# evenrose/CMDIAD

Measured on AMD Instinct MI355X. Metric: images/sec end-to-end (extract+distill+kNN score), higher is better.
Workload: dtype bf16; 1 GPU; configs[1]: DINO ViT-B/8 + Point-MAE predict (DoubleRGBPointFeatures: both modalities are extracted, this method has no distillation step at test time; the `mtfi_step` leg times the method that has one), 224x224 RGB + 24576-point clouds (1024 groups x 128), batch 32/GPU, bagel-sized banks (xyz 76518x768, rgb 19129x768); batch_per_gpu=32, rotating_input_batches=4, bank=single, hip_graphs=True, search_operands=bf16 (fp32 accumulate, exact fp32 re-score of the winner), weights=seeded random init (no checkpoints offline)

## Files before the change

### cmdiad_amd/csrc/mlp_fused.hip

```cpp
#include "gemm_core.h"
#include "launch.h"

namespace {

using namespace gemm;

constexpr int kC = 384, kHid = 1536, kBM = 128, kWaves = 8;
constexpr int kChunks = kHid / 64;
constexpr int kKT1 = kC / BK;
constexpr int kPer = kKT1 + kC / 64;
constexpr int kSlots = 6, kAhead = kSlots - 1;
static_assert(kPer % kSlots == 0, "the slot of a piece depends on its place in the chunk only");
constexpr int kPieceBytes = 64 * BK * 2;
constexpr int kXbWave = kKT1 * 16 * BK * 2;
constexpr int kHOff = kWaves * kXbWave;
constexpr int kRingOff = kHOff + kWaves * 2048;
constexpr int kLdsBytes = kRingOff + kSlots * kPieceBytes;
static_assert(kLdsBytes == 160 * 1024, "LDS budget");

struct MlpParams {
    int M;
    const bf16_t* xb;
    const float* row_scale;
    const bf16_t* w1;
    const float* b1;
    const bf16_t* w2;
    const float* b2;
    float* x;
    bf16_t* ln_xb;
    float* ln_part;
    const float* add2;
};

__device__ __forceinline__ void mlp_barrier() { asm volatile("s_barrier" ::: "memory"); }

__device__ __forceinline__ float half_row_sum8(float v)
{
    v += __builtin_bit_cast(float, __builtin_amdgcn_update_dpp(0, __builtin_bit_cast(int, v), 0xB1, 0xF, 0xF, false));
    v += __builtin_bit_cast(float, __builtin_amdgcn_update_dpp(0, __builtin_bit_cast(int, v), 0x4E, 0xF, 0xF, false));
    v += __builtin_bit_cast(float, __builtin_amdgcn_update_dpp(0, __builtin_bit_cast(int, v), 0x141, 0xF, 0xF, false));
    return v;
}

template <bool LN_OUT>
__global__ __launch_bounds__(512, 1) void pmae_mlp_fused_kernel(MlpParams p)
{
    extern __shared__ __attribute__((aligned(16))) char lds[];
    const int lane = threadIdx.x & 63, wave = __builtin_amdgcn_readfirstlane(threadIdx.x >> 6);
    const int g = lane >> 4, r16 = lane & 15;
    const int mw = (int)blockIdx.x * kBM + wave * 16;
    char* xs = lds + wave * kXbWave;
    char* hs = lds + kHOff + wave * 2048;
    char* ring = lds + kRingOff;

    float rsc;
    f32x4 b1v[4];
    auto load_b1 = [&](int c) {
        const float* bp = p.b1 + c * 64 + g * 4;
#pragma unroll
        for (int j = 0; j < 4; ++j) asm volatile("global_load_dwordx4 %0, %1, off" : "=v"(b1v[j]) : "v"(bp + j * 16) : "memory");
    };
    {
        const float* rp = p.row_scale + min(mw + r16, p.M - 1);
        asm volatile("global_load_dword %0, %1, off" : "=v"(rsc) : "v"(rp) : "memory");
    }
    load_b1(0);
    const int sw_chunk = (lane & 7) ^ (lane >> 3);
#pragma unroll
    for (int e = 0; e < 2; ++e) {
        const bf16_t* src = p.xb + (size_t)min(mw + e * 8 + (lane >> 3), p.M - 1) * kC + sw_chunk * 8;
#pragma unroll
        for (int s = 0; s < kKT1; ++s)
            __builtin_amdgcn_global_load_lds((const __attribute__((address_space(1))) void*)(src + s * BK),
                                             (__attribute__((address_space(3))) void*)(xs + s * 2048 + e * 1024), 16, 0, 0);
    }
    const char* w1l = reinterpret_cast<const char*>(p.w1 + (size_t)(wave * 8 + (lane >> 3)) * kC + sw_chunk * 8);
    const char* w2l = reinterpret_cast<const char*>(p.w2 + (size_t)(wave * 8 + (lane >> 3)) * kHid + sw_chunk * 8);
    auto issue = [&](int c, int q) {
        const char* src = q < kKT1 ? w1l + ((size_t)c * 64 * kC + q * BK) * 2 : w2l + ((size_t)(q - kKT1) * 64 * kHid + c * BK) * 2;
        __builtin_amdgcn_global_load_lds((const __attribute__((address_space(1))) void*)src,
                                         (__attribute__((address_space(3))) void*)(ring + (q % kSlots) * kPieceBytes + wave * 1024), 16, 0, 0);
    };
#pragma unroll
    for (int q = 0; q < kAhead; ++q) issue(0, q);
    asm volatile("s_waitcnt vmcnt(4)" ::: "memory");
    mlp_barrier();

    auto ldf = [&](const char* tile, int row, int kk) { return *reinterpret_cast<const bf16x8*>(tile + lds_off(row, kk * 4 + g)); };
    auto step = [&](const char* wt, const bf16x8& a0, const bf16x8& a1, f32x4 (&acc)[4]) {
        bf16x8 wf[2][4];
#pragma unroll
        for (int kk = 0; kk < 2; ++kk)
#pragma unroll
            for (int j = 0; j < 4; ++j) wf[kk][j] = ldf(wt, j * 16 + r16, kk);
        __builtin_amdgcn_s_setprio(1);
#pragma unroll
        for (int kk = 0; kk < 2; ++kk)
#pragma unroll
            for (int j = 0; j < 4; ++j) acc[j] = mfma16(wf[kk][j], kk ? a1 : a0, acc[j]);
        __builtin_amdgcn_s_setprio(0);
    };

    f32x4 acc2[kC / 64][4];
#pragma unroll
    for (int nb = 0; nb < kC / 64; ++nb)
#pragma unroll
        for (int j = 0; j < 4; ++j) acc2[nb][j] = f32x4{0.f, 0.f, 0.f, 0.f};

    for (int c = 0; c < kChunks; ++c) {
        f32x4 acc1[4];
#pragma unroll
        for (int j = 0; j < 4; ++j) acc1[j] = f32x4{0.f, 0.f, 0.f, 0.f};
        bf16x8 h0, h1;
#pragma unroll
        for (int q = 0; q < kPer; ++q) {
            const int qn = q + kAhead < kPer ? q + kAhead : q + kAhead - kPer;
            const int cn = q + kAhead < kPer ? c : c + 1;
            const bool more = cn < kChunks;
            if (q == 7 && more) load_b1(c + 1);
            if (more) issue(cn, qn);
            const char* wt = ring + (q % kSlots) * kPieceBytes;
            if (q < kKT1) step(wt, ldf(xs + q * 2048, r16, 0), ldf(xs + q * 2048, r16, 1), acc1);
            else step(wt, h0, h1, acc2[q - kKT1]);
            if (!more) asm volatile("s_waitcnt vmcnt(0)" ::: "memory");
            else if (q >= 7 && q <= 10) asm volatile("s_waitcnt vmcnt(8)" ::: "memory");
            else asm volatile("s_waitcnt vmcnt(4)" ::: "memory");
            mlp_barrier();
            if (q == kKT1 - 1) {
                __builtin_amdgcn_sched_barrier(0);
#pragma unroll
                for (int j = 0; j < 4; ++j) {
                    f32x4 v = __builtin_elementwise_fma(acc1[j], f32x4{rsc, rsc, rsc, rsc}, b1v[j]);
                    v = gelu_erf4(v);
                    const bf16x4 hv = {f2bf(v[0]), f2bf(v[1]), f2bf(v[2]), f2bf(v[3])};
                    *reinterpret_cast<bf16x4*>(hs + lds_off(r16, 2 * j + (g >> 1)) + (g & 1) * 8) = hv;
                }
                h0 = ldf(hs, r16, 0);
                h1 = ldf(hs, r16, 1);
            }
        }
    }

    RowStore32 rs;
    rs.init(hs, lane);
    const bool full = mw + 16 <= p.M;
    const int m0r = mw + rs.R;
    const int ma = min(m0r, p.M - 1), mb = min(m0r + 8, p.M - 1);
#pragma unroll
    for (int nb = 0; nb < kC / 64; ++nb) {
        const int n0 = nb * 64;
        f32x4 bj[4];
#pragma unroll
        for (int j = 0; j < 4; ++j) bj[j] = *reinterpret_cast<const f32x4*>(p.b2 + n0 + j * 16 + g * 4);
        f32x4 o0[2], o1[2];
#pragma unroll
        for (int ch = 0; ch < 2; ++ch) {
            const int col = n0 + ch * 32 + rs.u * 4;
            const f32x4 r0 = *reinterpret_cast<const f32x4*>(p.x + (size_t)ma * kC + col);
            const f32x4 r1 = *reinterpret_cast<const f32x4*>(p.x + (size_t)mb * kC + col);
            f32x4 a0 = {0.f, 0.f, 0.f, 0.f}, a1 = a0;
            if (LN_OUT && p.add2) {
                a0 = *reinterpret_cast<const f32x4*>(p.add2 + (size_t)ma * kC + col);
                a1 = *reinterpret_cast<const f32x4*>(p.add2 + (size_t)mb * kC + col);
            }
            rs.park(acc2[nb][2 * ch] + bj[2 * ch], acc2[nb][2 * ch + 1] + bj[2 * ch + 1]);
            f32x4 t0, t1;
            rs.fetch(t0, t1);
            o0[ch] = t0 + r0;
            o1[ch] = t1 + r1;
            if (LN_OUT && p.add2) { o0[ch] += a0; o1[ch] += a1; }
            if (full || m0r < p.M) *reinterpret_cast<f32x4*>(p.x + (size_t)m0r * kC + col) = o0[ch];
            if (full || m0r + 8 < p.M) *reinterpret_cast<f32x4*>(p.x + (size_t)(m0r + 8) * kC + col) = o1[ch];
            if constexpr (LN_OUT) {
                const bf16x4 v0 = {f2bf(o0[ch][0]), f2bf(o0[ch][1]), f2bf(o0[ch][2]), f2bf(o0[ch][3])};
                const bf16x4 v1 = {f2bf(o1[ch][0]), f2bf(o1[ch][1]), f2bf(o1[ch][2]), f2bf(o1[ch][3])};
                if (full || m0r < p.M) *reinterpret_cast<bf16x4*>(p.ln_xb + (size_t)m0r * kC + col) = v0;
                if (full || m0r + 8 < p.M) *reinterpret_cast<bf16x4*>(p.ln_xb + (size_t)(m0r + 8) * kC + col) = v1;
            }
        }
        if constexpr (LN_OUT) {
            float s0 = 0.f, s1 = 0.f;
#pragma unroll
            for (int ch = 0; ch < 2; ++ch)
#pragma unroll
                for (int q = 0; q < 4; ++q) { s0 += o0[ch][q]; s1 += o1[ch][q]; }
            s0 = half_row_sum8(s0);
            s1 = half_row_sum8(s1);
            const float c0 = s0 * (1.0f / 64), c1 = s1 * (1.0f / 64);
            float q0 = 0.f, q1 = 0.f;
#pragma unroll
            for (int ch = 0; ch < 2; ++ch)
#pragma unroll
                for (int q = 0; q < 4; ++q) {
                    const float d0 = o0[ch][q] - c0, d1 = o1[ch][q] - c1;
                    q0 = fmaf(d0, d0, q0);
                    q1 = fmaf(d1, d1, q1);
                }
            q0 = half_row_sum8(q0);
            q1 = half_row_sum8(q1);
            if (rs.u == 0) {
                float2* part = reinterpret_cast<float2*>(p.ln_part) + (size_t)nb * p.M;
                if (full || m0r < p.M) part[m0r] = make_float2(s0, q0);
                if (full || m0r + 8 < p.M) part[m0r + 8] = make_float2(s1, q1);
            }
        }
    }
}

}

int cmdiad_pmae_mlp_fused(float* x, const uint16_t* xb, const float* rstd, const uint16_t* w1, const float* b1, const uint16_t* w2,
                          const float* b2, int M, uint16_t* ln_xb, float* ln_part, const float* add2, cmdiad_stream_t stream)
{
    CMDIAD_REQUIRE(x && xb && rstd && w1 && b1 && w2 && b2 && M > 0, CMDIAD_ERR_ARG, "cmdiad_pmae_mlp_fused: null operand");
    CMDIAD_REQUIRE(aligned16(x) && aligned16(xb) && aligned16(w1) && aligned16(w2) && aligned16(b1) && aligned16(b2) && (!add2 || aligned16(add2)), CMDIAD_ERR_ARG,
                   "cmdiad_pmae_mlp_fused: operands must be 16-byte aligned");
    CMDIAD_REQUIRE(!ln_xb == !ln_part && (ln_xb || !add2) && (!ln_xb || (((uintptr_t)ln_xb & 7) == 0 && ((uintptr_t)ln_part & 7) == 0)),
                   CMDIAD_ERR_ARG, "cmdiad_pmae_mlp_fused: ln_xb and ln_part come together (8-byte aligned); add2 only with them");
    MlpParams p{M, (const bf16_t*)xb, rstd, (const bf16_t*)w1, b1, (const bf16_t*)w2, b2, x, (bf16_t*)ln_xb, ln_part, add2};
    const dim3 grid((unsigned)((M + kBM - 1) / kBM)), block(kWaves * 64);
    const int rc = ln_xb ? launch_lds<pmae_mlp_fused_kernel<true>>("cmdiad_pmae_mlp_fused", grid, block, kLdsBytes, (hipStream_t)stream, p)
                         : launch_lds<pmae_mlp_fused_kernel<false>>("cmdiad_pmae_mlp_fused", grid, block, kLdsBytes, (hipStream_t)stream, p);
    if (rc) return rc;
    CMDIAD_CHECK_LAUNCH();
    return CMDIAD_OK;
}
```

Before: 1593 images/s.

## Restructure fused Point-MAE MLP to 4 waves of 32 rows with register double-buffering

```diff
diff --git a/cmdiad_amd/csrc/mlp_fused.hip b/cmdiad_amd/csrc/mlp_fused.hip
--- a/cmdiad_amd/csrc/mlp_fused.hip
+++ b/cmdiad_amd/csrc/mlp_fused.hip
@@ -5,16 +5,19 @@
 
 using namespace gemm;
 
-constexpr int kC = 384, kHid = 1536, kBM = 128, kWaves = 8;
+constexpr int kC = 384, kHid = 1536, kBM = 128, kWaves = 4;
+constexpr int kRows = kBM / kWaves;
 constexpr int kChunks = kHid / 64;
 constexpr int kKT1 = kC / BK;
 constexpr int kPer = kKT1 + kC / 64;
-constexpr int kSlots = 6, kAhead = kSlots - 1;
-static_assert(kPer % kSlots == 0, "the slot of a piece depends on its place in the chunk only");
+constexpr int kSlots = 6;
+static_assert(kPer % kSlots == 0 && kPer % 2 == 0, "the slot and the fragment set of a piece depend on its place in the chunk only");
 constexpr int kPieceBytes = 64 * BK * 2;
-constexpr int kXbWave = kKT1 * 16 * BK * 2;
+constexpr int kXbTile = kRows * BK * 2;
+constexpr int kXbWave = kKT1 * kXbTile;
+constexpr int kHWave = kRows * BK * 2;
 constexpr int kHOff = kWaves * kXbWave;
-constexpr int kRingOff = kHOff + kWaves * 2048;
+constexpr int kRingOff = kHOff + kWaves * kHWave;
 constexpr int kLdsBytes = kRingOff + kSlots * kPieceBytes;
 static_assert(kLdsBytes == 160 * 1024, "LDS budget");
 
@@ -32,7 +35,20 @@
     const float* add2;
 };
 
-__device__ __forceinline__ void mlp_barrier() { asm volatile("s_barrier" ::: "memory"); }
+__device__ __forceinline__ void step_end(int n)
+{
+#define CMDIAD_STEP_END(N) asm volatile("s_waitcnt vmcnt(" #N ") lgkmcnt(0)\n\ts_barrier" ::: "memory")
+    __builtin_amdgcn_s_waitcnt(0xC07F);
+    switch (n) {
+    case 12: CMDIAD_STEP_END(12); break;
+    case 8: CMDIAD_STEP_END(8); break;
+    case 6: CMDIAD_STEP_END(6); break;
+    case 4: CMDIAD_STEP_END(4); break;
+    case 2: CMDIAD_STEP_END(2); break;
+    default: CMDIAD_STEP_END(0); break;
+    }
+#undef CMDIAD_STEP_END
+}
 
 __device__ __forceinline__ float half_row_sum8(float v)
 {
@@ -43,165 +59,228 @@
 }
 
 template <bool LN_OUT>
-__global__ __launch_bounds__(512, 1) void pmae_mlp_fused_kernel(MlpParams p)
+__global__ __launch_bounds__(kWaves * 64, 1) void pmae_mlp_fused_kernel(MlpParams p)
 {
     extern __shared__ __attribute__((aligned(16))) char lds[];
     const int lane = threadIdx.x & 63, wave = __builtin_amdgcn_readfirstlane(threadIdx.x >> 6);
     const int g = lane >> 4, r16 = lane & 15;
-    const int mw = (int)blockIdx.x * kBM + wave * 16;
+    const int mw = (int)blockIdx.x * kBM + wave * kRows;
     char* xs = lds + wave * kXbWave;
-    char* hs = lds + kHOff + wave * 2048;
+    char* hs = lds + kHOff + wave * kHWave;
     char* ring = lds + kRingOff;
 
-    float rsc;
+    float rsc[2];
     f32x4 b1v[4];
     auto load_b1 = [&](int c) {
         const float* bp = p.b1 + c * 64 + g * 4;
 #pragma unroll
         for (int j = 0; j < 4; ++j) asm volatile("global_load_dwordx4 %0, %1, off" : "=v"(b1v[j]) : "v"(bp + j * 16) : "memory");
     };
-    {
-        const float* rp = p.row_scale + min(mw + r16, p.M - 1);
-        asm volatile("global_load_dword %0, %1, off" : "=v"(rsc) : "v"(rp) : "memory");
+#pragma unroll
+    for (int rb = 0; rb < 2; ++rb) {
+        const float* rp = p.row_scale + min(mw + rb * 16 + r16, p.M - 1);
+        asm volatile("global_load_dword %0, %1, off" : "=v"(rsc[rb]) : "v"(rp) : "memory");
     }
     load_b1(0);
     const int sw_chunk = (lane & 7) ^ (lane >> 3);
 #pragma unroll
-    for (int e = 0; e < 2; ++e) {
+    for (int e = 0; e < kRows / 8; ++e) {
         const bf16_t* src = p.xb + (size_t)min(mw + e * 8 + (lane >> 3), p.M - 1) * kC + sw_chunk * 8;
 #pragma unroll
         for (int s = 0; s < kKT1; ++s)
             __builtin_amdgcn_global_load_lds((const __attribute__((address_space(1))) void*)(src + s * BK),
-                                             (__attribute__((address_space(3))) void*)(xs + s * 2048 + e * 1024), 16, 0, 0);
-    }
-    const char* w1l = reinterpret_cast<const char*>(p.w1 + (size_t)(wave * 8 + (lane >> 3)) * kC + sw_chunk * 8);
-    const char* w2l = reinterpret_cast<const char*>(p.w2 + (size_t)(wave * 8 + (lane >> 3)) * kHid + sw_chunk * 8);
+                                             (__attribute__((address_space(3))) void*)(xs + s * kXbTile + e * 1024), 16, 0, 0);
+    }
+    const char* w1l = reinterpret_cast<const char*>(p.w1 + (size_t)(wave * 16 + (lane >> 3)) * kC + sw_chunk * 8);
+    const char* w2l = reinterpret_cast<const char*>(p.w2 + (size_t)(wave * 16 + (lane >> 3)) * kHid + sw_chunk * 8);
     auto issue = [&](int c, int q) {
         const char* src = q < kKT1 ? w1l + ((size_t)c * 64 * kC + q * BK) * 2 : w2l + ((size_t)(q - kKT1) * 64 * kHid + c * BK) * 2;
-        __builtin_amdgcn_global_load_lds((const __attribute__((address_space(1))) void*)src,
-                                         (__attribute__((address_space(3))) void*)(ring + (q % kSlots) * kPieceBytes + wave * 1024), 16, 0, 0);
-    };
-#pragma unroll
-    for (int q = 0; q < kAhead; ++q) issue(0, q);
-    asm volatile("s_waitcnt vmcnt(4)" ::: "memory");
-    mlp_barrier();
-
-    auto ldf = [&](const char* tile, int row, int kk) { return *reinterpret_cast<const bf16x8*>(tile + lds_off(row, kk * 4 + g)); };
-    auto step = [&](const char* wt, const bf16x8& a0, const bf16x8& a1, f32x4 (&acc)[4]) {
-        bf16x8 wf[2][4];
+        const size_t ld8 = (size_t)(q < kKT1 ? kC : kHid) * 8 * 2;
+#pragma unroll
+        for (int e = 0; e < 2; ++e)
+            __builtin_amdgcn_global_load_lds((const __attribute__((address_space(1))) void*)(src + e * ld8),
+                                             (__attribute__((address_space(3))) void*)(ring + (q % kSlots) * kPieceBytes + wave * 2048 + e * 1024),
+                                             16, 0, 0);
+    };
+#pragma unroll
+    for (int q = 0; q < kSlots; ++q) issue(0, q);
+    step_end(8);
+
+    typedef const __attribute__((address_space(3))) char* lds_cptr;
+    lds_cptr wb[2], xb_[2], hb[2];
+#pragma unroll
+    for (int kk = 0; kk < 2; ++kk) {
+        wb[kk] = (lds_cptr)(ring + lds_off(r16, kk * 4 + g));
+        xb_[kk] = (lds_cptr)(xs + lds_off(r16, kk * 4 + g));
+        hb[kk] = (lds_cptr)(hs + lds_off(r16, kk * 4 + g));
+    }
+    auto ldf = [&](lds_cptr base, int off) { return *reinterpret_cast<const __attribute__((address_space(3))) bf16x8*>(base + off); };
+    bf16x8 wf[2][2][4], af[2][2][2], hf[2][2];
+    auto read_w = [&](int set, int slot) {
 #pragma unroll
         for (int kk = 0; kk < 2; ++kk)
 #pragma unroll
-            for (int j = 0; j < 4; ++j) wf[kk][j] = ldf(wt, j * 16 + r16, kk);
-        __builtin_amdgcn_s_setprio(1);
-#pragma unroll
-        for (int kk = 0; kk < 2; ++kk)
-#pragma unroll
-            for (int j = 0; j < 4; ++j) acc[j] = mfma16(wf[kk][j], kk ? a1 : a0, acc[j]);
-        __builtin_amdgcn_s_setprio(0);
-    };
-
-    f32x4 acc2[kC / 64][4];
-#pragma unroll
-    for (int nb = 0; nb < kC / 64; ++nb)
-#pragma unroll
-        for (int j = 0; j < 4; ++j) acc2[nb][j] = f32x4{0.f, 0.f, 0.f, 0.f};
-
-    for (int c = 0; c < kChunks; ++c) {
-        f32x4 acc1[4];
-#pragma unroll
-        for (int j = 0; j < 4; ++j) acc1[j] = f32x4{0.f, 0.f, 0.f, 0.f};
-        bf16x8 h0, h1;
+            for (int j = 0; j < 4; ++j) wf[set][kk][j] = ldf(wb[kk], slot * kPieceBytes + j * 2048);
+    };
+    auto read_x = [&](int set, int s) {
+#pragma unroll
+        for (int rb = 0; rb < 2; ++rb)
+#pragma unroll
+            for (int kk = 0; kk < 2; ++kk) af[set][rb][kk] = ldf(xb_[kk], s * kXbTile + rb * 2048);
+    };
+    read_w(0, 0);
+    read_x(0, 0);
+    step_end(8);
+
+    f32x4 acc2[2][kC / 64][4];
+#pragma unroll
+    for (int rb = 0; rb < 2; ++rb)
+#pragma unroll
+        for (int nb = 0; nb < kC / 64; ++nb)
+#pragma unroll
+            for (int j = 0; j < 4; ++j) acc2[rb][nb][j] = f32x4{0.f, 0.f, 0.f, 0.f};
+
+    auto chunk = [&](int c, auto last_t) {
+        constexpr bool last = decltype(last_t)::value;
+        f32x4 acc1[2][4];
+#pragma unroll
+        for (int rb = 0; rb < 2; ++rb)
+#pragma unroll
+            for (int j = 0; j < 4; ++j) acc1[rb][j] = f32x4{0.f, 0.f, 0.f, 0.f};
 #pragma unroll
         for (int q = 0; q < kPer; ++q) {
-            const int qn = q + kAhead < kPer ? q + kAhead : q + kAhead - kPer;
-            const int cn = q + kAhead < kPer ? c : c + 1;
+            const int cur = q & 1, nxt = cur ^ 1;
+            const int qn = (q + kSlots) % kPer;
+            const int cn = q + kSlots < kPer ? c : c + 1;
             const bool more = cn < kChunks;
             if (q == 7 && more) load_b1(c + 1);
             if (more) issue(cn, qn);
-            const char* wt = ring + (q % kSlots) * kPieceBytes;
-            if (q < kKT1) step(wt, ldf(xs + q * 2048, r16, 0), ldf(xs + q * 2048, r16, 1), acc1);
-            else step(wt, h0, h1, acc2[q - kKT1]);
-            if (!more) asm volatile("s_waitcnt vmcnt(0)" ::: "memory");
-            else if (q >= 7 && q <= 10) asm volatile("s_waitcnt vmcnt(8)" ::: "memory");
-            else asm volatile("s_waitcnt vmcnt(4)" ::: "memory");
-            mlp_barrier();
+            if (q < kKT1) {
+                read_w(nxt, (q + 1) % kSlots);
+                if (q + 1 < kKT1) read_x(nxt, q + 1);
+#pragma unroll
+                for (int kk = 0; kk < 2; ++kk)
+#pragma unroll
+                    for (int rb = 0; rb < 2; ++rb)
+#pragma unroll
+                        for (int j = 0; j < 4; ++j) acc1[rb][j] = mfma16(wf[cur][kk][j], af[cur][rb][kk], acc1[rb][j]);
+                if (q + 1 < kKT1) {
+#pragma unroll
+                    for (int i = 0; i < 6; ++i) {
+                        __builtin_amdgcn_sched_group_barrier(0x008, 2, 0);
+                        __builtin_amdgcn_sched_group_barrier(0x100, 2, 0);
+                    }
+                } else {
+#pragma unroll
+                    for (int i = 0; i < 8; ++i) {
+                        __builtin_amdgcn_sched_group_barrier(0x008, 2, 0);
+                        __builtin_amdgcn_sched_group_barrier(0x100, 1, 0);
+                    }
+                }
+            } else {
+                if (q + 1 == kPer) read_x(nxt, 0);
+#pragma unroll
+                for (int kk = 0; kk < 2; ++kk)
+#pragma unroll
+                    for (int rb = 0; rb < 2; ++rb)
+#pragma unroll
+                        for (int j = 0; j < 4; ++j) {
+                            asm volatile("v_mfma_f32_16x16x32_bf16 %0, %1, %2, %0" : "+a"(acc2[rb][q - kKT1][j]) : "v"(wf[cur][kk][j]), "v"(hf[rb][kk]) : "memory");
+                            const int n = kk * 8 + rb * 4 + j;
+                            if (n & 1) wf[nxt][n >> 3][(n >> 1) & 3] = ldf(wb[n >> 3], ((q + 1) % kSlots) * kPieceBytes + ((n >> 1) & 3) * 2048);
+                        }
+            }
             if (q == kKT1 - 1) {
-                __builtin_amdgcn_sched_barrier(0);
-#pragma unroll
-                for (int j = 0; j < 4; ++j) {
-                    f32x4 v = __builtin_elementwise_fma(acc1[j], f32x4{rsc, rsc, rsc, rsc}, b1v[j]);
-                    v = gelu_erf4(v);
-                    const bf16x4 hv = {f2bf(v[0]), f2bf(v[1]), f2bf(v[2]), f2bf(v[3])};
-                    *reinterpret_cast<bf16x4*>(hs + lds_off(r16, 2 * j + (g >> 1)) + (g & 1) * 8) = hv;
-                }
-                h0 = ldf(hs, r16, 0);
-                h1 = ldf(hs, r16, 1);
+#pragma unroll
+                for (int rb = 0; rb < 2; ++rb)
+#pragma unroll
+                    for (int j = 0; j < 4; ++j) {
+                        f32x4 v = __builtin_elementwise_fma(acc1[rb][j], f32x4{rsc[rb], rsc[rb], rsc[rb], rsc[rb]}, b1v[j]);
+                        v = gelu_erf4(v);
+                        const bf16x4 hv = {f2bf(v[0]), f2bf(v[1]), f2bf(v[2]), f2bf(v[3])};
+                        *reinterpret_cast<bf16x4*>(hs + lds_off(rb * 16 + r16, 2 * j + (g >> 1)) + (g & 1) * 8) = hv;
+                    }
+#pragma unroll
+                for (int rb = 0; rb < 2; ++rb)
+#pragma unroll
+                    for (int kk = 0; kk < 2; ++kk) hf[rb][kk] = ldf(hb[kk], rb * 2048);
+            }
+            if (!last) {
+                step_end(q >= 7 && q <= 9 ? 12 : 8);
+            } else {
+                const int left = kPer - 1 - (q + 2);
+                step_end(left >= 4 ? 8 : left > 0 ? 2 * left : 0);
             }
         }
-    }
+    };
+    for (int c = 0; c < kChunks - 1; ++c) chunk(c, std::false_type());
+    chunk(kChunks - 1, std::true_type());
+    asm volatile("s_nop 15\n\ts_nop 15" ::: "memory");
 
     RowStore32 rs;
     rs.init(hs, lane);
-    const bool full = mw + 16 <= p.M;
-    const int m0r = mw + rs.R;
-    const int ma = min(m0r, p.M - 1), mb = min(m0r + 8, p.M - 1);
-#pragma unroll
-    for (int nb = 0; nb < kC / 64; ++nb) {
-        const int n0 = nb * 64;
-        f32x4 bj[4];
-#pragma unroll
-        for (int j = 0; j < 4; ++j) bj[j] = *reinterpret_cast<const f32x4*>(p.b2 + n0 + j * 16 + g * 4);
-        f32x4 o0[2], o1[2];
-#pragma unroll
-        for (int ch = 0; ch < 2; ++ch) {
-            const int col = n0 + ch * 32 + rs.u * 4;
-            const f32x4 r0 = *reinterpret_cast<const f32x4*>(p.x + (size_t)ma * kC + col);
-            const f32x4 r1 = *reinterpret_cast<const f32x4*>(p.x + (size_t)mb * kC + col);
-            f32x4 a0 = {0.f, 0.f, 0.f, 0.f}, a1 = a0;
-            if (LN_OUT && p.add2) {
-                a0 = *reinterpret_cast<const f32x4*>(p.add2 + (size_t)ma * kC + col);
-                a1 = *reinterpret_cast<const f32x4*>(p.add2 + (size_t)mb * kC + col);
-            }
-            rs.park(acc2[nb][2 * ch] + bj[2 * ch], acc2[nb][2 * ch + 1] + bj[2 * ch + 1]);
-            f32x4 t0, t1;
-            rs.fetch(t0, t1);
-            o0[ch] = t0 + r0;
-            o1[ch] = t1 + r1;
-            if (LN_OUT && p.add2) { o0[ch] += a0; o1[ch] += a1; }
-            if (full || m0r < p.M) *reinterpret_cast<f32x4*>(p.x + (size_t)m0r * kC + col) = o0[ch];
-            if (full || m0r + 8 < p.M) *reinterpret_cast<f32x4*>(p.x + (size_t)(m0r + 8) * kC + col) = o1[ch];
+#pragma unroll
+    for (int rb = 0; rb < 2; ++rb) {
+        const bool full = mw + rb * 16 + 16 <= p.M;
+        const int m0r = mw + rb * 16 + rs.R;
+        const int ma = min(m0r, p.M - 1), mb = min(m0r + 8, p.M - 1);
+#pragma unroll
+        for (int nb = 0; nb < kC / 64; ++nb) {
+            const int n0 = nb * 64;
+            f32x4 bj[4];
+#pragma unroll
+            for (int j = 0; j < 4; ++j) bj[j] = *reinterpret_cast<const f32x4*>(p.b2 + n0 + j * 16 + g * 4);
+            f32x4 o0[2], o1[2];
+#pragma unroll
+            for (int ch = 0; ch < 2; ++ch) {
+                const int col = n0 + ch * 32 + rs.u * 4;
+                const f32x4 r0 = *reinterpret_cast<const f32x4*>(p.x + (size_t)ma * kC + col);
+                const f32x4 r1 = *reinterpret_cast<const f32x4*>(p.x + (size_t)mb * kC + col);
+                f32x4 a0 = {0.f, 0.f, 0.f, 0.f}, a1 = a0;
+                if (LN_OUT && p.add2) {
+                    a0 = *reinterpret_cast<const f32x4*>(p.add2 + (size_t)ma * kC + col);
+                    a1 = *reinterpret_cast<const f32x4*>(p.add2 + (size_t)mb * kC + col);
+                }
+                rs.park(acc2[rb][nb][2 * ch] + bj[2 * ch], acc2[rb][nb][2 * ch + 1] + bj[2 * ch + 1]);
+                f32x4 t0, t1;
+                rs.fetch(t0, t1);
+                o0[ch] = t0 + r0;
+                o1[ch] = t1 + r1;
+                if (LN_OUT && p.add2) { o0[ch] += a0; o1[ch] += a1; }
+                if (full || m0r < p.M) *reinterpret_cast<f32x4*>(p.x + (size_t)m0r * kC + col) = o0[ch];
+                if (full || m0r + 8 < p.M) *reinterpret_cast<f32x4*>(p.x + (size_t)(m0r + 8) * kC + col) = o1[ch];
+                if constexpr (LN_OUT) {
+                    const bf16x4 v0 = {f2bf(o0[ch][0]), f2bf(o0[ch][1]), f2bf(o0[ch][2]), f2bf(o0[ch][3])};
+                    const bf16x4 v1 = {f2bf(o1[ch][0]), f2bf(o1[ch][1]), f2bf(o1[ch][2]), f2bf(o1[ch][3])};
+                    if (full || m0r < p.M) *reinterpret_cast<bf16x4*>(p.ln_xb + (size_t)m0r * kC + col) = v0;
+                    if (full || m0r + 8 < p.M) *reinterpret_cast<bf16x4*>(p.ln_xb + (size_t)(m0r + 8) * kC + col) = v1;
+                }
+            }
             if constexpr (LN_OUT) {
-                const bf16x4 v0 = {f2bf(o0[ch][0]), f2bf(o0[ch][1]), f2bf(o0[ch][2]), f2bf(o0[ch][3])};
-                const bf16x4 v1 = {f2bf(o1[ch][0]), f2bf(o1[ch][1]), f2bf(o1[ch][2]), f2bf(o1[ch][3])};
-                if (full || m0r < p.M) *reinterpret_cast<bf16x4*>(p.ln_xb + (size_t)m0r * kC + col) = v0;
-                if (full || m0r + 8 < p.M) *reinterpret_cast<bf16x4*>(p.ln_xb + (size_t)(m0r + 8) * kC + col) = v1;
-            }
-        }
-        if constexpr (LN_OUT) {
-            float s0 = 0.f, s1 = 0.f;
-#pragma unroll
-            for (int ch = 0; ch < 2; ++ch)
-#pragma unroll
-                for (int q = 0; q < 4; ++q) { s0 += o0[ch][q]; s1 += o1[ch][q]; }
-            s0 = half_row_sum8(s0);
-            s1 = half_row_sum8(s1);
-            const float c0 = s0 * (1.0f / 64), c1 = s1 * (1.0f / 64);
-            float q0 = 0.f, q1 = 0.f;
-#pragma unroll
-            for (int ch = 0; ch < 2; ++ch)
-#pragma unroll
-                for (int q = 0; q < 4; ++q) {
-                    const float d0 = o0[ch][q] - c0, d1 = o1[ch][q] - c1;
-                    q0 = fmaf(d0, d0, q0);
-                    q1 = fmaf(d1, d1, q1);
+                float s0 = 0.f, s1 = 0.f;
+#pragma unroll
+                for (int ch = 0; ch < 2; ++ch)
+#pragma unroll
+                    for (int q = 0; q < 4; ++q) { s0 += o0[ch][q]; s1 += o1[ch][q]; }
+                s0 = half_row_sum8(s0);
+                s1 = half_row_sum8(s1);
+                const float c0 = s0 * (1.0f / 64), c1 = s1 * (1.0f / 64);
+                float q0 = 0.f, q1 = 0.f;
+#pragma unroll
+                for (int ch = 0; ch < 2; ++ch)
+#pragma unroll
+                    for (int q = 0; q < 4; ++q) {
+                        const float d0 = o0[ch][q] - c0, d1 = o1[ch][q] - c1;
+                        q0 = fmaf(d0, d0, q0);
+                        q1 = fmaf(d1, d1, q1);
+                    }
+                q0 = half_row_sum8(q0);
+                q1 = half_row_sum8(q1);
+                if (rs.u == 0) {
+                    float2* part = reinterpret_cast<float2*>(p.ln_part) + (size_t)nb * p.M;
+                    if (full || m0r < p.M) part[m0r] = make_float2(s0, q0);
+                    if (full || m0r + 8 < p.M) part[m0r + 8] = make_float2(s1, q1);
                 }
-            q0 = half_row_sum8(q0);
-            q1 = half_row_sum8(q1);
-            if (rs.u == 0) {
-                float2* part = reinterpret_cast<float2*>(p.ln_part) + (size_t)nb * p.M;
-                if (full || m0r < p.M) part[m0r] = make_float2(s0, q0);
-                if (full || m0r + 8 < p.M) part[m0r + 8] = make_float2(s1, q1);
             }
         }
     }
```

Result: no change. 1600 images/s, median of 6 (+0.4%).
